# Corleno/Nonstationary_Multivariate_Gaussian_Process

Hardware: AMD Instinct MI355X
Metric: log-posterior evals/sec (N=2048, D=3 nonseparable GP) (higher is better)
Workload: dtype f64

## Files before the change

nonstationary_multivariate_gaussian_process_amd/csrc/nmgp_chol.hip:

```cpp
#include "nmgp_internal.h"
#include <cstring>

namespace nmgpk {

static inline int cdiv_c(long long a, long long b) { return (int)((a + b - 1) / b); }

typedef double v4d __attribute__((ext_vector_type(4)));

#define SY_BM 128
#define SY_BK 16
#define SY_LD (SY_BM + 16)
#define SY_SB 8

__device__ __forceinline__ int clamp_row_pair(int r, int rows) {
    int rc = r < rows - 1 ? r : rows - 2;
    return rc < 0 ? 0 : rc;
}

__device__ __forceinline__ double fast_recip(double p) {
    double x = __builtin_amdgcn_rcp(p);
    double e = fma(-p, x, 1.0);
    x = fma(x, e, x);
    e = fma(-p, x, 1.0);
    x = fma(x, e, x);
// ... 47 lines not shown
    potf2_step<KC, 2>(a, colbuf, pivs, nb, info, goff, r, g, tid);
    potf2_step<KC, 3>(a, colbuf, pivs, nb, info, goff, r, g, tid);
}

__device__ __forceinline__ void potf2_body(double* __restrict__ A, int lda, int nb, int* __restrict__ info, int goff, int tid,
                                           double (*colbuf)[64], double* pivs) {
    const int r = tid & 63, g = (tid >> 6) & 3;
    double a[16];
#pragma unroll
    for (int kk = 0; kk < 16; ++kk) {
        const int c = 4 * kk + g;
        double v = (r == c) ? 1.0 : 0.0;
        if (r < nb && c <= r) v = A[(size_t)c * lda + r];
        a[kk] = v;
    }
    if (tid < 64) pivs[tid] = 1.0;
    if (g == 0) colbuf[0][r] = a[0];
    __syncthreads();
#define PF(K) potf2_steps4<K>(a, colbuf, pivs, nb, info, goff, r, g, tid)
    PF(0); PF(1); PF(2); PF(3); PF(4); PF(5); PF(6); PF(7); PF(8); PF(9); PF(10); PF(11); PF(12); PF(13); PF(14); PF(15);
#undef PF
    __syncthreads();
#pragma unroll
    for (int kk = 0; kk < 16; ++kk) {
        const int c = 4 * kk + g;
        if (r < nb && c <= r) A[(size_t)c * lda + r] = a[kk] * rsqrt(pivs[c]);
    }
}

typedef double v2d __attribute__((ext_vector_type(2)));
typedef int v4i __attribute__((ext_vector_type(4)));

__device__ __forceinline__ void syrk_fused_first_block(double* lds, const v4d (&acc)[2][2][2], bool owner, int wj,
                                                       double* __restrict__ C, int ldc, int* __restrict__ info, int goff);

#define SY_SMEM (4 * SY_BK * SY_LD)
#define SCHUR_PATCH (32 * 33)
#define SY_SCHUR_SMEM (8 * SCHUR_PATCH + 6 * 256)
static_assert(SY_SCHUR_SMEM >= SY_SMEM && SY_SCHUR_SMEM * 8 * 2 <= 160 * 1024, "Schur epilogue LDS");

template <int M>
__device__ __forceinline__ double svc_schur_value(double sigma2, int a, int b, bool rc, const double* __restrict__ Lr, double il2,
                                                  const double* __restrict__ Lc, double kv, double nai, double gcb) {
    constexpr int UR = M <= 3 ? 8 : 1;
    const double gra = sigma2 * Lr[a * (a + 1) / 2] * il2;
    double s = 0.0;
#pragma unroll UR
    for (int q = 1; q <= b; ++q) s += Lr[a * (a + 1) / 2 + q] * Lc[b * (b + 1) / 2 + q];
    double v = kv * s;
    if (rc) v += sigma2 * ((a == b ? 1.0 : 0.0) + Lr[a * (a + 1) / 2] * Lr[b * (b + 1) / 2] * il2);
    v += gra * nai * gcb;
    return v;
}

template <int M, bool ALLB>
__device__ __forceinline__ void svc_schur_entries(const SchurEpi& e, double sigma2, int r, const double* __restrict__ Lr, double il2,
                                                  int c, double kv, double nai, const double* gc) {
    constexpr int T = M * (M + 1) / 2;
    constexpr int UR = M <= 3 ? 8 : 1;
    const size_t Ns = (size_t)e.N;
    const double* __restrict__ Lc = e.Lv + (size_t)c * T;
    const double lcc = M <= 4 ? 0.0 : Lc[0];
#pragma unroll UR
    for (int a = 1; a < M; ++a) {
#pragma unroll UR
        for (int b = 1; b <= (ALLB ? a : a - 1); ++b) {
            const double gcb = M <= 4 ? gc[b - 1] : sigma2 * Lc[b * (b + 1) / 2] / (lcc * lcc);
// ... 71 lines not shown
                        const double* Lc = e.Lv + (size_t)c * T_;
                        P[il * 33 + jl] = svc_schur_value<M>(sigma2, 2, 1, false, Lc, gc[M - 1], Lr, kv, nai, gt[(128 + r - row0) * GS]);
                    }
                } else {
                    svc_schur_entries<M, false>(e, sigma2, r, Lr, il2, c, kv, nai, gc);
                }
            }
        }
        __builtin_amdgcn_wave_barrier();
    }
}

template <int M>
__device__ __forceinline__ void svc_schur_yrow(const SchurEpi& e, int i) {
    constexpr int T = M * (M + 1) / 2;
    if (i >= e.N) return;
    const size_t Ns = (size_t)e.N;
    const int n1 = (M - 1) * e.N;
    const double sigma2 = exp(e.tse[0]);
    const double* Li = e.Lv + (size_t)i * T;
    const double l00 = Li[0];
    const double il2 = 1.0 / (l00 * l00);
    const double vi = e.y[i] / l00;
    const double r = vi - (sigma2 * il2) * e.u[i];
#pragma unroll
    for (int a = 1; a < M; ++a) e.S[((size_t)(a - 1) * Ns + i) * e.ld + n1] = e.y[(size_t)a * Ns + i] - Li[a * (a + 1) / 2] * r;
}

template <int SM = 0>
__device__ __forceinline__ void syrk_tile_fast(const double* __restrict__ A, int lda, double* __restrict__ C, int ldc, int K,
                                               int row0, int col0, bool diag, int kt0, bool beta0, int ncw, int yrow,
                                               int nyr, double* sA0, double* sB0, bool skip00 = false,
                                               int* __restrict__ finfo = nullptr, int fgoff = 0, bool mirror = false,
                                               int fresh0 = 0x7fffffff, const SchurEpi* se = nullptr) {
    constexpr int BK = 16;
    constexpr int SBUF = BK * SY_LD;
    const int tid = threadIdx.x, lane = tid & 63, w = tid >> 6;
    const int wi = w & 1, wj = w >> 1;
    const int l15 = lane & 15, l4 = lane >> 4;
    const int rp = tid & 63, cg = tid >> 6;
    const int offA = (cg * lda + row0 + 2 * rp) * 8, offB = (cg * lda + col0 + 2 * rp) * 8;
    const __amdgpu_buffer_rsrc_t rsrc = __builtin_amdgcn_make_buffer_rsrc((void*)A, 0, 0x7fffffff, 0x00020000);
    const int gstep = BK * lda * 8, ghalf = 8 * lda * 8;
    int soff = kt0 * gstep;
    const bool has_y = diag && yrow >= 0;
    const bool ywave = has_y && wi == 0 && wj >= 2;
    const int offY = ((tid & 15) * lda + yrow + (tid >> 4)) * 8;
    double* sY = sB0;
    v4i ra0, ra1, rb0, rb1;
    double ry = 0.0;
    auto gload = [&]() {
        ra0 = __builtin_amdgcn_raw_buffer_load_b128(rsrc, offA, soff, 0);
        ra1 = __builtin_amdgcn_raw_buffer_load_b128(rsrc, offA, soff + ghalf, 0);
        if (!diag) {
            rb0 = __builtin_amdgcn_raw_buffer_load_b128(rsrc, offB, soff, 0);
            rb1 = __builtin_amdgcn_raw_buffer_load_b128(rsrc, offB, soff + ghalf, 0);
        }
        if (has_y && tid < 16 * nyr) {
            typedef int v2i __attribute__((ext_vector_type(2)));
            const v2i t2 = __builtin_amdgcn_raw_buffer_load_b64(rsrc, offY, soff, 0);
            ry = __builtin_bit_cast(double, t2);
        }
        soff += gstep;
    };
    double* wA = sA0 + cg * SY_LD + 2 * rp;
    double* wB = sB0 + cg * SY_LD + 2 * rp;
    auto sstore = [&](int buf) {
// ... 138 lines not shown
#pragma unroll
            for (int r = 0; r < 4; ++r) {
                const int i = row0 + wi * 64 + 32 * p + 2 * l15;
                const int j = col0 + wj * 32 + 2 * (l4 + 4 * r) + tj;
                if (diag && j > i + 1) continue;
                double2 c;
                c.x = -acc[p][0][tj][r];
                c.y = -acc[p][1][tj][r];
                if (diag && j == i + 1) C[(size_t)j * ldc + i + 1] = c.y;
                else *reinterpret_cast<double2*>(&C[(size_t)j * ldc + i]) = c;
            }
    }
    if (mirror && active) {
        double* T = sA0 + w * (32 * 33);
        const int jl = lane & 31, ih = lane >> 5;
#pragma unroll
        for (int p = 0; p < 2; ++p) {
#pragma unroll
            for (int sx = 0; sx < 2; ++sx)
#pragma unroll
                for (int tj = 0; tj < 2; ++tj)
#pragma unroll
                    for (int r = 0; r < 4; ++r) T[(2 * l15 + sx) * 33 + 2 * (l4 + 4 * r) + tj] = -acc[p][sx][tj][r];
            const int rowm = col0 + wj * 32 + jl;
#pragma unroll
            for (int q = 0; q < 16; ++q) {
                const int il = 2 * q + ih;
                const int colm = row0 + wi * 64 + 32 * p + il;
                const double v = T[il * 33 + jl];
                if (colm > rowm) C[(size_t)colm * ldc + rowm] = v;
            }
        }
    }
    if (finfo != nullptr) syrk_fused_first_block(sA0, acc, fowner, wj, C, ldc, finfo, fgoff);
}

template <int NWJ, int BK, int SM = 0>
__device__ __forceinline__ void syrk_tile_body(const double* __restrict__ A, int lda, double* __restrict__ C, int ldc, int mrows,
                                               int ncols, int K, long long bstride, long long cstride, int ktri, int swz,
                                               int nbatch, int bx, int by, int bz0, double* sAb, double* sBb,
                                               int tri_row0 = 0x7fffffff, int tri_k0 = 0, int* __restrict__ finfo = nullptr,
                                               int fistride = 0, int fgoff = 0, const SchurEpi* sep = nullptr) {
    const int nyr = (ktri >> 2) & 31;
    const bool skipq = (ktri & 128) != 0;
    const bool mirror = (ktri & 512) != 0;
    const bool rowmajor = (ktri & 1024) != 0;
    const int yrow = nyr ? mrows : -1;
    (void)rowmajor;
    ktri &= 1;
    const int fresh0 = tri_row0 == 0x7fffffff ? 0x7fffffff : tri_row0 + tri_k0;
    constexpr int NT = 128 * NWJ;
    constexpr int CW = 128 / NWJ;
    constexpr int TJ = CW / 16;
    constexpr int NQ = (64 * BK) / NT;
    constexpr int CGS = NT / 64;
    double (*sA)[BK * SY_LD] = reinterpret_cast<double (*)[BK * SY_LD]>(sAb);
    double (*sB)[BK * SY_LD] = reinterpret_cast<double (*)[BK * SY_LD]>(sBb);
    int bi = bx, bj = by;
    int bz = bz0;
    if (swz) {
        const int t = bx, q = t >> 3;
        const int tiles_pm = swz > 0 ? swz : -swz;
        const long long g = swz > 0 ? ((long long)(q >> 6) * 8 + (t & 7)) * 64 + (q & 63) : (long long)t;
        int idx;
        if (finfo != nullptr) {
            if (g >= (long long)tiles_pm * nbatch) return;
            if (g < nbatch) {
                bz = (int)g;
                idx = 0;
            } else {
                const long long g2 = g - nbatch;
                bz = (int)(g2 / (tiles_pm - 1));
                idx = 1 + (int)(g2 - (long long)bz * (tiles_pm - 1));
            }
        } else {
            bz = (int)(g / tiles_pm);
            if (bz >= nbatch) return;
            idx = (int)(g - (long long)bz * tiles_pm);
        }
// ... 41 lines not shown
    bi = __builtin_amdgcn_readfirstlane(bi);
    bj = __builtin_amdgcn_readfirstlane(bj);
    bz = __builtin_amdgcn_readfirstlane(bz);
    A += (size_t)bz * bstride;
    C += (size_t)bz * cstride;
    SchurEpi se{};
    if constexpr (SM > 0) {
        static_assert(NWJ == 4 && BK == 16, "the Schur epilogue assumes 8 waves of 64 x 32");
        constexpr int T = SM * (SM + 1) / 2;
        se = *sep;
        se.x += (size_t)(bz / se.cps) * se.xstride;
        se.y += (size_t)(bz / se.cps) * se.ystride;
        se.ell += (size_t)bz * se.N;
        se.Lv += (size_t)bz * se.N * T;
        se.tse += (size_t)bz * ((size_t)se.N * (1 + T) + 1);
        se.u += (size_t)bz * se.N;
        se.S += (size_t)bz * se.bstride;
    }
    const bool diag = (bi == bj);
    const int tid = threadIdx.x, lane = tid & 63, w = tid >> 6;
    const int wi = w & 1, wj = w >> 1;
    const int row0 = bi * SY_BM, col0 = bj * SY_BM;
    if constexpr (NWJ == 4 && BK == 16) {
        const int ncw = ncols - col0 >= SY_BM ? SY_BM : ncols - col0;
        if (row0 + SY_BM <= mrows && (ncw == SY_BM || ncw == 64) && col0 + SY_BM <= mrows && (K & 31) == 0 &&
            (long long)(K + 16) * lda * 8 < 0x7fff0000LL) {
            int kt0f = ktri ? row0 / BK : 0;
            if (row0 >= tri_row0) {
                const int z = (row0 - tri_row0 - tri_k0) / BK;
                kt0f = z > 0 ? (z & ~1) : 0;
            }
            syrk_tile_fast<SM>(A, lda, C, ldc, K, row0, col0, diag, kt0f, ktri != 0, ncw, yrow, nyr, &sA[0][0], &sB[0][0],
                               skipq && bi == 0 && bj == 0, (finfo != nullptr && bi == 0 && bj == 0) ? finfo + (size_t)bz * fistride : nullptr,
                               fgoff, mirror, fresh0, &se);
            return;
        }
    }
    const int rp = tid & 63, cg = tid >> 6;
    double2 ra[NQ], rb[NQ];

    const int ri = row0 + 2 * rp, rj = col0 + 2 * rp;
    const int ric = clamp_row_pair(ri, mrows), rjc = clamp_row_pair(rj, mrows);
    const bool ix = ri < mrows, iy = ri + 1 < mrows, jx = rj < mrows, jy = rj + 1 < mrows;
    const bool ish = ix && (ric != ri), jsh = jx && (rjc != rj);
    auto gload = [&](int k0) {
#pragma unroll
        for (int q = 0; q < NQ; ++q) {
            const int kc = k0 + cg + CGS * q;
            const double* colp = A + (size_t)(kc < K ? kc : K - 1) * lda;
            ra[q] = *reinterpret_cast<const double2*>(colp + ric);
            if (!diag) rb[q] = *reinterpret_cast<const double2*>(colp + rjc);
        }
    };
    auto sstore = [&](int buf, int k0) {
#pragma unroll
        for (int q = 0; q < NQ; ++q) {
            const int kl = cg + CGS * q;
            const bool kin = (k0 + kl) < K;
            double2 va, vb;
            va.x = (kin && ix) ? (ish ? ra[q].y : ra[q].x) : 0.0;
            va.y = (kin && iy) ? ra[q].y : 0.0;
            *reinterpret_cast<double2*>(&sA[buf][kl * SY_LD + 2 * rp]) = va;
            if (!diag) {
                vb.x = (kin && jx) ? (jsh ? rb[q].y : rb[q].x) : 0.0;
                vb.y = (kin && jy) ? rb[q].y : 0.0;
                *reinterpret_cast<double2*>(&sB[buf][kl * SY_LD + 2 * rp]) = vb;
            }
// ... 355 lines not shown
            for (int r = 0; r < 4; ++r) {
                const int a = l4 + 4 * r, b = l15;
                Sr[r] = (a >= b) ? P.S[(16 * i + b) * PB_LD + 16 * i + a] : P.S[(16 * i + a) * PB_LD + 16 * i + b];
            }
#pragma unroll
            for (int kk = 0; kk < 4; ++kk) Sr = __builtin_amdgcn_mfma_f64_16x16x4f64(-Xown[kk], Xown[kk], Sr, 0, 0, 0);
        } else if (w < 3 && i < 4) {
            Xown = solve_rows(q, i);
            for (int j = q + 1; j <= i; ++j) {
                const v4d xj = (j == i) ? Xown : solve_rows(q, j);
                v4d acc;
#pragma unroll
                for (int reg = 0; reg < 4; ++reg) acc[reg] = P.S[(16 * j + l4 + 4 * reg) * PB_LD + 16 * i + l15];
#pragma unroll
                for (int kk = 0; kk < 4; ++kk) acc = __builtin_amdgcn_mfma_f64_16x16x4f64(-xj[kk], Xown[kk], acc, 0, 0, 0);
#pragma unroll
                for (int reg = 0; reg < 4; ++reg) P.S[(16 * j + l4 + 4 * reg) * PB_LD + 16 * i + l15] = acc[reg];
            }
        }
    }
    __syncthreads();
}

__device__ __forceinline__ void potf2b_store(double* __restrict__ A, int lda, int nb, const Potf2Lds& P, int tid, int nthreads) {
    for (int idx = tid; idx < 4096; idx += nthreads) {
        const int r = idx & 63, c = idx >> 6;
        if (r < nb && c < nb) {
            if (c <= r) A[(size_t)c * lda + r] = P.S[c * PB_LD + r];
            else if ((c >> 4) == (r >> 4)) A[(size_t)c * lda + r] = P.Einv[c >> 4][c & 15][r & 15];
        }
    }
}

__device__ __forceinline__ void syrk_fused_first_block(double* lds, const v4d (&acc)[2][2][2], bool owner, int wj,
                                                       double* __restrict__ C, int ldc, int* __restrict__ info, int goff) {
    static_assert(sizeof(Potf2Lds) <= 4 * SY_BK * SY_LD * sizeof(double), "the block's LDS must fit the operand buffers");
    Potf2Lds& P = *reinterpret_cast<Potf2Lds*>(lds);
    const int tid = threadIdx.x, lane = tid & 63;
    const int l15 = lane & 15, l4 = lane >> 4;
    for (int idx = tid; idx < 4096; idx += (int)blockDim.x) {
        const int r = idx & 63, c = idx >> 6;
        if (c > r) P.S[c * PB_LD + r] = 0.0;
    }
    if (owner) {
#pragma unroll
        for (int p = 0; p < 2; ++p)
#pragma unroll
            for (int sx = 0; sx < 2; ++sx)
#pragma unroll
                for (int tj = 0; tj < 2; ++tj)
#pragma unroll
                    for (int r = 0; r < 4; ++r) {
                        const int i = 32 * p + 2 * l15 + sx;
                        const int j = 32 * wj + 2 * (l4 + 4 * r) + tj;
                        if (i >= j) P.S[j * PB_LD + i] = -acc[p][sx][tj][r];
                    }
    }
    __syncthreads();
    potf2b_core_mfma(P, info, goff);
    potf2b_store(C, ldc, 64, P, tid, (int)blockDim.x);
}

__global__ __launch_bounds__(256) void k_potf2_64b(double* __restrict__ A, int lda, int nb, int* __restrict__ info,
                                                    int goff, long long bstride, int istride) {
    A += (size_t)blockIdx.x * bstride;
    info += (size_t)blockIdx.x * istride;
    __shared__ Potf2Lds P;
    const int tid = threadIdx.x;
#pragma unroll
    for (int k = 0; k < 16; ++k) {
        const int idx = tid + 256 * k;
        const int r = idx & 63, c = idx >> 6;
        double v = (r == c) ? 1.0 : 0.0;
        if (r < nb && c <= r) v = A[(size_t)c * lda + r];
        P.S[c * PB_LD + r] = v;
    }
    __syncthreads();
    potf2b_core_mfma(P, info, goff);
    potf2b_store(A, lda, nb, P, tid, 256);
}

static void potf2_64(hipStream_t s, double* A, int lda, int nb, int* info, int goff, int batch, long long bstride,
                     int istride, bool precise) {
    if (precise)
        NMGP_LAUNCH(k_potf2_64, dim3(batch), dim3(256), 0, s, A, lda, nb, info, goff, bstride, istride);
    else
        NMGP_LAUNCH(k_potf2_64b, dim3(batch), dim3(256), 0, s, A, lda, nb, info, goff, bstride, istride);
}

#define SS_LD 80
__global__ __launch_bounds__(256) void k_syrk_small(const double* __restrict__ A, int lda, double* __restrict__ C, int ldc,
                                                     int mrows, int ncols, int K, long long bstride, int tiles_pm, int nbatch,
                                                     int tri_row0, int tri_k0, int* __restrict__ info, int istride, int goff) {
// ... 109 lines not shown
            if (c > r) P.S[c * PB_LD + r] = 0.0;
        }
        if (active) {
#pragma unroll
            for (int tj = 0; tj < 2; ++tj)
#pragma unroll
                for (int ti = 0; ti < 2; ++ti)
#pragma unroll
                    for (int r = 0; r < 4; ++r) {
                        const int i = wi * 32 + ti * 16 + l15;
                        const int j = wj * 32 + tj * 16 + l4 + 4 * r;
                        if (i >= j) P.S[j * PB_LD + i] = acc[tj][ti][r];
                    }
        }
        __syncthreads();
        potf2b_core_mfma(P, info + (size_t)bz * istride, goff);
        potf2b_store(C, ldc, 64, P, tid, 256);
        return;
    }
    if (active) {
#pragma unroll
        for (int tj = 0; tj < 2; ++tj)
#pragma unroll
            for (int ti = 0; ti < 2; ++ti)
#pragma unroll
                for (int r = 0; r < 4; ++r) {
                    const int i = row0 + wi * 32 + ti * 16 + l15;
                    const int j = col0 + wj * 32 + tj * 16 + l4 + 4 * r;
                    if (i < mrows && j < ncols && i >= j) C[(size_t)j * ldc + i] = acc[tj][ti][r];
                }
    }
}

bool syrk_lower(hipStream_t s, const double* A, int lda, double* C, int ldc, int mrows, int ncols, int K, int batch,
                long long bstride, long long cstride, int ktri, int tri_row0, int tri_k0, int* finfo, int fistride, int goff,
                const SyrkHook* hook) {
    if (mrows <= 0 || ncols <= 0 || K <= 0) return false;
    const SyrkPlan pl = syrk_plan(lda, ldc, mrows, ncols, K, batch, ktri, false, tri_row0 != kNoTriRows);
    const long long cs = cstride < 0 ? bstride : cstride;
    void* tok = nullptr;
    if (hook && hook->begin) {
        const double elems = (double)ncols * mrows - 0.5 * (double)ncols * (ncols - 1);
        tok = hook->begin(hook->user, s, 2.0 * K * elems * batch, 8.0 * batch * (2.0 * elems + (double)mrows * K));
    }
    bool fused;
    if (!ktri && K >= 128 && batch <= 16 && (long long)pl.tiles * batch <= switches().syrk_small_max && cs == bstride &&
        (lda & 1) == 0 && mrows >= 2) {
        const int gx = (mrows + 63) / 64, gy = (ncols + 63) / 64;
        int tiles = 0;
        for (int bj = 0; bj < gy; ++bj) tiles += gx - bj > 0 ? gx - bj : 0;
        fused = finfo != nullptr && mrows >= 64 && ncols >= 64;
        NMGP_LAUNCH(k_syrk_small, dim3((unsigned)(tiles * batch)), dim3(256), 0, s, A, lda, C, ldc, mrows, ncols, K, bstride, tiles,
                    batch, tri_row0, tri_k0, fused ? finfo : (int*)nullptr, fistride, goff);
    } else {
        fused = finfo != nullptr && !ktri && cs == bstride && pl.mrows >= SY_BM && (ncols >= SY_BM || ncols == 64) &&
                (K & 31) == 0 && (long long)(K + 16) * lda * 8 < 0x7fff0000LL;
        SyrkPlan pf = pl;
        if (fused && pf.swz == 0) {
            pf.grid = dim3((unsigned)((long long)pf.tiles * batch), 1, 1);
            pf.swz = -pf.tiles;
        }
        NMGP_LAUNCH(k_syrk_lower, pf.grid, dim3(512), 0, s, A, lda, C, ldc, pf.mrows, ncols, K, bstride, cs, pf.kflags,
                    pf.swz, batch, tri_row0, tri_k0, fused ? finfo : (int*)nullptr, fistride, goff);
    }
    if (tok && hook->end) hook->end(hook->user, tok);
    return fused;
}

int syrk_schur(hipStream_t s, const double* X, int lda, int N, int M, int batch, const SchurEpi& e) {
    if (N <= 0) return 0;
    if (M < 2 || M > 8) return NMGP_E_UNSUPPORTED;
    const SyrkPlan pl = syrk_plan(lda, lda, N, N, N, batch, 2, false);
    switch (M) {
#define SCHUR_CASE(m) \
        case m: NMGP_LAUNCH(k_syrk_schur<m>, pl.grid, dim3(512), 0, s, X, lda, pl.mrows, e.bstride, pl.kflags, pl.swz, batch, e); break;
        SCHUR_CASE(2) SCHUR_CASE(3) SCHUR_CASE(4) SCHUR_CASE(5) SCHUR_CASE(6) SCHUR_CASE(7) SCHUR_CASE(8)
#undef SCHUR_CASE
    }
    return 0;
}


template <int SRC>
__device__ inline double quad_bcast(double v) {
    constexpr int ctrl = SRC | (SRC << 2) | (SRC << 4) | (SRC << 6);
    int lo = __double2loint(v), hi = __double2hiint(v);
    lo = __builtin_amdgcn_mov_dpp(lo, ctrl, 0xF, 0xF, true);
    hi = __builtin_amdgcn_mov_dpp(hi, ctrl, 0xF, 0xF, true);
    return __hiloint2double(hi, lo);
}

template <int KC, int GC>
__device__ __forceinline__ void trsm_step(double (&x)[16], const double (*Lm)[65], const double* rinv, int g) {
    constexpr int c = 4 * KC + GC;
    double xc = x[KC] * rinv[c];
    xc = quad_bcast<GC>(xc);
    if (g == GC) x[KC] = xc;
    double t[16];
#pragma unroll
// ... 482 lines not shown
    __syncthreads();
    PS_STAMP(5);
    if (isC) {
#pragma unroll
        for (int sg = 0; sg < 4; ++sg)
#pragma unroll
            for (int kk = 0; kk < 4; ++kk)
#pragma unroll
                for (int q = 0; q < 4; ++q) {
                    const double a = -Xs[(16 * q + l15) * PS_XLD + 16 * sg + 4 * kk + l4];
                    Un[q] = __builtin_amdgcn_mfma_f64_16x16x4f64(a, Tk[sg][kk], Un[q], 0, 0, 0);
                }
    }
    Potf2Lds& P = *reinterpret_cast<Potf2Lds*>(smem);
    __syncthreads();
    if (isC) {
#pragma unroll
        for (int q = 0; q < 4; ++q)
#pragma unroll
            for (int r = 0; r < 4; ++r) {
                const int rr = 16 * w + l15, cc = 16 * q + 4 * r + l4;
                P.S[cc * PB_LD + rr] = (cc <= rr) ? Un[q][r] : 0.0;
            }
    }
    __syncthreads();
    PS_STAMP(6);
    potf2b_core_mfma(P, info + (size_t)by * istride, ck + 64);
    PS_STAMP(7);
    potf2b_store(A + (size_t)(ck + 64) * lda + (ck + 64), lda, 64, P, tid, 512);
    PS_STAMP(8);
#undef PS_STAMP
}

__global__ void k_set_row(double* __restrict__ A, int lda, int row, const double* __restrict__ v, int n,
                          long long bstride, long long vstride, int cps) {
    int j = blockIdx.x * blockDim.x + threadIdx.x;
    if (j < n) A[(size_t)blockIdx.y * bstride + (size_t)j * lda + row] = v[(size_t)(blockIdx.y / cps) * vstride + j];
}
void set_row(hipStream_t s, double* A, int lda, int row, const double* v, int n, int batch, long long bstride,
             long long vstride, int cps) {
    NMGP_LAUNCH(k_set_row, dim3(cdiv_c(n, 256), batch), dim3(256), 0, s, A, lda, row, v, n, bstride, vstride, cps < 1 ? 1 : cps);
}
__global__ void k_get_row(const double* __restrict__ A, int lda, int row, double* __restrict__ v, int n,
                          long long bstride, long long vstride) {
    int j = blockIdx.x * blockDim.x + threadIdx.x;
    if (j < n) v[(size_t)blockIdx.y * vstride + j] = A[(size_t)blockIdx.y * bstride + (size_t)j * lda + row];
}
void get_row(hipStream_t s, const double* A, int lda, int row, double* v, int n, int batch, long long bstride,
             long long vstride) {
    NMGP_LAUNCH(k_get_row, dim3(cdiv_c(n, 256), batch), dim3(256), 0, s, A, lda, row, v, n, bstride, vstride);
}

struct Factorisation {
    hipStream_t s, s2;
    double* A;
    int lda, n, extra, xtri;
    int* info;
    int batch;
    long long bs;
    int is;
    bool precise;
    const SyrkHook* hook;
    long long* stamps;
    bool block_done = false;

    double* at(int row, int col) const { return A + (size_t)col * lda + row; }
    int active_rows(int cend) const { return n + extra + (cend < xtri ? cend : xtri); }
    bool take_block_done() {
        const bool done = block_done;
        block_done = false;
        return done;
    }

    void update(hipStream_t st, int c0, int k, int c1, int ncols, int fuse_width) {
        const bool fuse = fuse_width >= 64 && !precise;
        const bool done = syrk_lower(st, at(c1, c0), lda, at(c1, c1), lda, active_rows(c0 + k) - c1, ncols, k, batch, bs, -1, 0,
                                     xtri > 0 ? n + extra - c1 : kNoTriRows, c0, fuse ? info : nullptr, is, c1, hook);
        if (fuse) block_done = done;
    }

    void block_solve(int c0, int w) {
        if (!take_block_done()) potf2_64(s, at(c0, c0), lda, w, info, c0, batch, bs, is, precise);
        trsm_64(s, at(c0, c0), lda, w, at(c0 + w, c0), lda, active_rows(c0 + w) - (c0 + w), batch, bs, precise);
    }

    void fused_steps(int c0, int w, bool leaf) {
        if (!take_block_done()) potf2_64(s, at(c0, c0), lda, 64, info, c0, batch, bs, is, precise);
        const int nk = w / 64;
        for (int k = 0; k < nk; ++k) {
            const int ck = c0 + 64 * k;
            const int m_act = active_rows(ck + 64);
            const int rows = m_act - (ck + 64);
            if (rows <= 0) continue;
            const int has_prev = k > 0, has_next = k + 1 < nk;
            const int T = 1 + (rows > 64 ? cdiv_c(rows - 64, 128) : 0);
            SyrkPlan pl;
            const int u_m = m_act - (ck + 128), u_n = c0 + w - (ck + 128);
            if (has_prev && u_m > 0 && u_n > 0) pl = syrk_plan(lda, lda, u_m, u_n, 64, 1, 0, true);
            const int pre = (ck + 192 <= c0 + w) ? 1 : 0;
            if (pre) pl.kflags |= 128;
            long long* st = stamps ? stamps + (size_t)(ck / 64) * 16 : nullptr;
            const int un_fresh = xtri > 0 ? n + extra + (has_prev ? ck - 64 : ck) : kNoTriRows;
            const int u_tri = xtri > 0 ? n + extra - 64 * NMGP_XTRI_SEED_BLOCKS : kNoTriRows;
            if (leaf && pl.tiles == 0 && !pre && nk == 2) {
                if (k == 0)
                    NMGP_LAUNCH((k_panel_step<1, 4>), dim3((unsigned)(T * batch)), dim3(512), 0, s, A, lda, ck, 0, 1, m_act, c0 + w, bs, info,
                                is, T, 0, 0, 0, 0, batch, 0, un_fresh, u_tri, st);
                else
                    NMGP_LAUNCH((k_panel_step<2, 6>), dim3((unsigned)(T * batch)), dim3(512), 0, s, A, lda, ck, 1, 0, m_act, c0 + w, bs, info,
                                is, T, 0, 0, 0, 0, batch, 0, un_fresh, u_tri, st);
            } else {
                NMGP_LAUNCH((k_panel_step<0, 2>), dim3((unsigned)((T + pl.tiles) * batch)), dim3(512), 0, s, A, lda, ck, has_prev, has_next, m_act,
                            c0 + w, bs, info, is, T, pl.mrows, u_n, pl.kflags, pl.tiles, batch, pre, un_fresh, u_tri, st);
            }
        }
    }

    void panel_rl(int c0, int w) {
        for (int j0 = c0; j0 < c0 + w; j0 += 64) {
            const int jb = (c0 + w - j0 < 64) ? (c0 + w - j0) : 64;
            block_solve(j0, jb);
            update(s, j0, jb, j0 + jb, c0 + w - (j0 + jb), c0 + w - (j0 + jb));
        }
    }

    enum Leaf {
        kBlockSolve,
        kFusedSteps,
        kLeaf128
    };
    void panel_halving(int c0, int w, int base, Leaf leaf) {
        if (w <= base) {
            if (leaf == kBlockSolve || (leaf == kLeaf128 && w != 128)) block_solve(c0, w);
            else fused_steps(c0, w, leaf == kLeaf128);
            return;
        }
        int h = ((w / 2 + 63) / 64) * 64;
        if (h >= w) h = ((w - 1) / 64) * 64;
        panel_halving(c0, h, base, leaf);
        update(s, c0, h, c0 + h, w - h, w - h);
        panel_halving(c0 + h, w - h, base, leaf);
    }

    void panel(int c0, int w) {
        const Switches& sw = switches();
        const bool mfma_ok = w > 0 && (w % 64 == 0) && (lda % 2 == 0) && !precise;
        const bool small = sw.fused_max_batch >= 0 ? batch <= sw.fused_max_batch : (long long)batch * n <= 73728;
        const int rec_min_batch = 4;
        if (mfma_ok && (sw.panel == Switches::kFused || (sw.panel == Switches::kAuto && small)))
            panel_halving(c0, w, fused_base(w), kFusedSteps);
        else if (mfma_ok && sw.panel == Switches::kAuto && batch >= rec_min_batch && w >= 128)
            panel_halving(c0, w, 128, kLeaf128);
        else if (sw.panel == Switches::kRl || (sw.panel != Switches::kRec && batch < rec_min_batch))
            panel_rl(c0, w);
        else
            panel_halving(c0, w, 64, kBlockSolve);
    }
    int fused_base(int w) const {
        if (switches().fused_base >= 64) return switches().fused_base;
        if (w > 256 && (batch >= 16 || (xtri > 0 && batch >= 5))) return 256;
        return w;
    }

    void run(int nb1, hipEvent_t* ev) {
        const bool la = (s2 != nullptr && ev != nullptr && n > 2 * nb1 && batch <= switches().la_max_batch && !precise);
        if (!la) {
            for (int c0 = 0; c0 < n; c0 += nb1) {
                const int w1 = (n - c0 < nb1) ? (n - c0) : nb1;
                const int c1 = c0 + w1;
                panel(c0, w1);
                update(s, c0, w1, c1, n - c1, n - c1 < nb1 ? n - c1 : nb1);
            }
            return;
        }
        hipEventRecord(ev[0], s);
        hipStreamWaitEvent(s2, ev[0], 0);
        int k = 0;
        bool prevB = false;
        for (int c0 = 0; c0 < n; c0 += nb1, ++k) {
            const int w1 = (n - c0 < nb1) ? (n - c0) : nb1;
            const int c1 = c0 + w1;
            const int w1n = (c1 < n) ? ((n - c1 < nb1) ? (n - c1) : nb1) : 0;
            const int c2 = c1 + w1n;
            hipEvent_t evPanel = ev[1 + 2 * k], evB = ev[2 + 2 * k];
            panel(c0, w1);
            if (c1 >= n) break;
            if (prevB) hipStreamWaitEvent(s, ev[2 + 2 * (k - 1)], 0);
            update(s, c0, w1, c1, w1n, w1n);
            hipEventRecord(evPanel, s);
            prevB = false;
            if (c2 < n) {
                hipStreamWaitEvent(s2, evPanel, 0);
                update(s2, c0, w1, c2, n - c2, 0);
                hipEventRecord(evB, s2);
                prevB = true;
            }
        }
        if (prevB) hipStreamWaitEvent(s, ev[2 + 2 * (k - 1)], 0);
    }
};

void potrf_lower(hipStream_t s, hipStream_t s2, hipEvent_t* ev, double* A, int lda, int n, int extra, int xtri,
                 int nb1, int* info, int batch, long long bstride, int istride, const SyrkHook* hook, int precise) {
    if (nb1 <= 0)
        nb1 = (batch >= 16 && n >= 4096) ? 2048
              : (((batch >= 4 && n >= 4096) || (batch >= 32 && n >= 2048)) && (long long)batch * n > 73728) ? 1024 : 512;
    const int nsteps = (n + 63) / 64;
    Factorisation f{s, s2, A, lda, n, extra, xtri, info, batch, bstride, istride, precise != 0, hook, g_step_stamps.begin(s, nsteps)};
    f.run(nb1, ev);
    g_step_stamps.dump(s, nsteps);
}

static_assert(SY_BM + 2 * SY_BK - 2 <= 64 * NMGP_XTRI_SEED_BLOCKS, "update tiles of L^-T rows would read left of the seeded band");
static_assert(NMGP_XTRI_SEED_BLOCKS == 3, "k_panel_step (u_tri) and k_xtri_seed's grid (4 column blocks per row block) assume three seeded blocks");
__global__ __launch_bounds__(256) void k_xtri_seed(double* __restrict__ A, int lda, int row0, int n, int pad,
                                                    long long bstride) {
    A += (size_t)blockIdx.z * bstride;
    const int lane = threadIdx.x & 63, w = threadIdx.x >> 6;
    if (blockIdx.x == gridDim.x - 1) {
        for (int c = blockIdx.y * 256 + threadIdx.x; c < n; c += 256 * gridDim.y)
            for (int q = 0; q < pad; ++q) A[(size_t)c * lda + row0 + q] = 0.0;
// ... 18 lines not shown
```

nonstationary_multivariate_gaussian_process_amd/csrc/nmgp_internal.h:

```cpp
#pragma once

#include <hip/hip_runtime.h>
#include <rocblas/rocblas.h>
#include <rocsolver/rocsolver.h>

#include <cmath>
#include <cstdio>
#include <cstdlib>
#include <cstring>
#include <map>
#include <string>
#include <utility>
#include <vector>

#include "nmgp.h"

#define NMGP_JITTER 1e-6
#define NMGP_PRECISION 1e-6

struct DevBuf {
    double* p = nullptr;
    size_t cap = 0;
};

// ... 315 lines not shown
void pred_rows_reduce(hipStream_t st, const double* A, int ld, int n, int R0, int zrow, int E, double* part, double* mean,
                      double* colsq);
void svc_predvar(hipStream_t st, const double* Lstar, const double* colsq, int S, int M, const double* tse,
                 double* var);
void sep_crossvec(hipStream_t st, int mode, const double* x, const double* sig, const double* ell, int N,
                  const double* xs, const double* tl_star, const double* ts_star, double sig0, double l0, int S,
                  double* KX);
void sep_predict(hipStream_t st, const double* Cq, const double* a, const double* wB, const double* VB, int M,
                 const double* wK, int N, double sigma2, const double* Bdiag, const double* kss, bool strict_clip, int S,
                 double* mean, double* var);
void sep_predict_chol(hipStream_t st, const double* dots, const double* sqs, const double* wB, const double* VB, int M, double sigma2,
                      const double* Bdiag, const double* kss, bool strict_clip, int S, double* mean, double* var);
void cols_to_rows(hipStream_t st, const double* KX, int N, int S, double* A, int ld, int R0, int batch, long long bstride);
void sep_star(hipStream_t st, const double* proj, int S, double mu_l, double mu_s, double* tl_star, double* ts_star,
              double* kss);
void add_diag(hipStream_t s, double* A, int ld, int n, double v);
void rotate_y(hipStream_t s, const double* Y, const double* VB, int N, int M, double* yt);
void sep_blocks(hipStream_t s, const double* K, const double* wB, const double* sigma2p, int N, int M, double* out,
                int ldo, long long bstride);
#define NMGP_SEP_TR_G 128
int sep_traces(hipStream_t s, const double* Cneg, const double* K, const double* alpha, int N, int M, double* out);
void weighted_sum_lower(hipStream_t s, const double* Cneg, const double* wB, int N, int M, double* C);
void sep_prep_b(hipStream_t s, const double* pars, long long P, const double* Y, const double* small, int small_per, int N, int M,
                double* ell, double* sig, double* yt, int B);
void sep_blocks_b(hipStream_t s, const double* x, const double* ell, const double* sig, const double* small, int small_per, int N, int M,
                  double* S, int ldo, long long bstride, double* Kout, int B);
void sep_reduce_b(hipStream_t s, const double* Cneg, const double* K, const double* alpha, const double* small, int small_per, int N,
                  int M, int G, double* C, double* out, double* xi, int B);
void sep_adjoint_b(hipStream_t s, const double* x, const double* ell, const double* sig, const double* U, const double* small,
                   int small_per, int M, const double* C, int N, double* part, double* g, int B);
void two_col_rhs_b(hipStream_t s, const double* pars, long long P, double mu_a, double mu_b, int N, double* R, int B);
void ps_rows_reduce(hipStream_t s, const double* A, int ld, long long bstride, int n, int R0, int zrow, int E, double* part,
                    int batch, double* dots, double* sqs, long long ostride, long long o0);
bool syrk_lower(hipStream_t s, const double* A, int lda, double* C, int ldc, int mrows, int ncols, int K, int batch,
                long long bstride, long long cstride = -1, int ktri = 0, int tri_row0 = 0x7fffffff, int tri_k0 = 0,
                int* finfo = nullptr, int fistride = 0, int goff = 0, const SyrkHook* hook = nullptr);
struct SchurEpi {
    const double* x;
    const double* ell;
    const double* Lv;
    const double* tse;
    const double* y;
    const double* u;
    double* S;
    int ld;
    int N;
    int xstride;
    int cps;
    long long ystride;
    long long bstride;
};
int syrk_schur(hipStream_t s, const double* X, int lda, int N, int M, int batch, const SchurEpi& e);
void identity_rows(hipStream_t s, double* A, int lda, int row0, int n, int pad, int batch = 1, long long bstride = 0);
void set_row(hipStream_t s, double* A, int lda, int row, const double* v, int n, int batch, long long bstride,
             long long vstride, int cps = 1);
void get_row(hipStream_t s, const double* A, int lda, int row, double* v, int n, int batch, long long bstride,
             long long vstride);
void potrf_lower(hipStream_t s, hipStream_t s2, hipEvent_t* ev, double* A, int lda, int n, int extra, int xtri,
                 int nb1, int* info, int batch, long long bstride, int istride, const SyrkHook* hook = nullptr,
                 int precise = 0);

}
```

Measured before the change: 1694.

## Add fused 128-column leaf kernels for throughput Cholesky panels

Adds k_leaf_diag128 and k_leaf128, which factor a 128-wide diagonal block and solve the panel rows below it with f64 MFMA triangular solves in a single launch. The SYRK epilogue can now factor the whole 128-column diagonal block instead of only 64, and a width-256 leaf is split into two 128 leaves with an update between them. This is meant to cut kernel launches and global round trips in the batched throughput schedule. It adds a lot of control flow and larger LDS use, and it only applies when the kLeaf128 schedule is selected.

Result: faster. 1714, median of 6 (+1.2%).

```diff
diff --git a/nonstationary_multivariate_gaussian_process_amd/csrc/nmgp_chol.hip b/nonstationary_multivariate_gaussian_process_amd/csrc/nmgp_chol.hip
--- a/nonstationary_multivariate_gaussian_process_amd/csrc/nmgp_chol.hip
+++ b/nonstationary_multivariate_gaussian_process_amd/csrc/nmgp_chol.hip
@@ -103,7 +103,8 @@
 typedef int v4i __attribute__((ext_vector_type(4)));
 
 __device__ __forceinline__ void syrk_fused_first_block(double* lds, const v4d (&acc)[2][2][2], bool owner, int wj,
-                                                       double* __restrict__ C, int ldc, int* __restrict__ info, int goff);
+                                                       double* __restrict__ C, int ldc, int* __restrict__ info, int goff,
+                                                       bool whole128);
 
 #define SY_SMEM (4 * SY_BK * SY_LD)
 #define SCHUR_PATCH (32 * 33)
@@ -241,7 +242,7 @@
                                                int row0, int col0, bool diag, int kt0, bool beta0, int ncw, int yrow,
                                                int nyr, double* sA0, double* sB0, bool skip00 = false,
                                                int* __restrict__ finfo = nullptr, int fgoff = 0, bool mirror = false,
-                                               int fresh0 = 0x7fffffff, const SchurEpi* se = nullptr) {
+                                               int fresh0 = 0x7fffffff, const SchurEpi* se = nullptr, bool f128 = false) {
     constexpr int BK = 16;
     constexpr int SBUF = BK * SY_LD;
     const int tid = threadIdx.x, lane = tid & 63, w = tid >> 6;
@@ -446,7 +447,7 @@
             }
         }
     }
-    if (finfo != nullptr) syrk_fused_first_block(sA0, acc, fowner, wj, C, ldc, finfo, fgoff);
+    if (finfo != nullptr) syrk_fused_first_block(sA0, acc, fowner, wj, C, ldc, finfo, fgoff, f128);
 }
 
 template <int NWJ, int BK, int SM = 0>
@@ -459,6 +460,7 @@
     const bool skipq = (ktri & 128) != 0;
     const bool mirror = (ktri & 512) != 0;
     const bool rowmajor = (ktri & 1024) != 0;
+    const bool f128 = (ktri & 2048) != 0;
     const int yrow = nyr ? mrows : -1;
     (void)rowmajor;
     ktri &= 1;
@@ -566,7 +568,7 @@
             }
             syrk_tile_fast<SM>(A, lda, C, ldc, K, row0, col0, diag, kt0f, ktri != 0, ncw, yrow, nyr, &sA[0][0], &sB[0][0],
                                skipq && bi == 0 && bj == 0, (finfo != nullptr && bi == 0 && bj == 0) ? finfo + (size_t)bz * fistride : nullptr,
-                               fgoff, mirror, fresh0, &se);
+                               fgoff, mirror, fresh0, &se, f128);
             return;
         }
     }
@@ -988,8 +990,116 @@
     }
 }
 
+__device__ __forceinline__ void trsm_ops_load(const double* __restrict__ L, int lda, int tid, double (&ot)[5]) {
+#pragma unroll
+    for (int j = 0; j < 5; ++j) {
+        const int idx = tid + 512 * j;
+        const int blk = idx >> 8, kk = (idx >> 6) & 3, l = idx & 63;
+        const int rr = l & 15, kc = 4 * kk + (l >> 4);
+        double v;
+        if (blk < 6) {
+            const int q = blk == 0 ? 1 : (blk < 3 ? 2 : 3);
+            const int pp = blk == 0 ? 0 : (blk < 3 ? blk - 1 : blk - 3);
+            v = -L[(size_t)(16 * pp + kc) * lda + 16 * q + rr];
+        } else {
+            const int q = blk - 6;
+            if (kc < rr) v = L[(size_t)(16 * q + rr) * lda + 16 * q + kc];
+            else if (kc == rr) v = 1.0 / L[(size_t)(16 * q + rr) * lda + 16 * q + rr];
+            else v = 0.0;
+        }
+        ot[j] = v;
+    }
+}
+__device__ __forceinline__ void trsm_ops_store(double* ops, int tid, const double (&ot)[5]) {
+#pragma unroll
+    for (int j = 0; j < 5; ++j) {
+        const int idx = tid + 512 * j;
+        const int blk = idx >> 8, kk = (idx >> 6) & 3, l = idx & 63;
+        ops[(blk * 64 + l) * 4 + kk] = ot[j];
+    }
+}
+__device__ __forceinline__ void trsm_solve64(v4d (&T)[4], const v4d* ops, int lane) {
+#pragma unroll
+    for (int pp = 0; pp < 4; ++pp) {
+        const v4d ai = ops[(6 + pp) * 64 + lane];
+        v4d x0 = {0.0, 0.0, 0.0, 0.0};
+#pragma unroll
+        for (int kk = 0; kk < 4; ++kk) x0 = __builtin_amdgcn_mfma_f64_16x16x4f64(ai[kk], T[pp][kk], x0, 0, 0, 0);
+        T[pp] = x0;
+#pragma unroll
+        for (int kk = 0; kk < 4; ++kk)
+#pragma unroll
+            for (int q = pp + 1; q < 4; ++q) {
+                const double a = reinterpret_cast<const double*>(&ops[((q == 1 ? 0 : (q == 2 ? 1 : 3)) + pp) * 64 + lane])[kk];
+                T[q] = __builtin_amdgcn_mfma_f64_16x16x4f64(a, T[pp][kk], T[q], 0, 0, 0);
+            }
+    }
+}
+
+#define LD_XLD 66
+#define LD_SMEM_DOUBLES (2560 + 64 * LD_XLD)
+static_assert(sizeof(Potf2Lds) <= LD_SMEM_DOUBLES * sizeof(double), "the factorisation's LDS aliases the solve's");
+__device__ __forceinline__ void leaf_diag_lower(double* __restrict__ D, int lda, int* __restrict__ info, int goff, double* smem) {
+    const int tid = threadIdx.x, lane = tid & 63, w = tid >> 6;
+    const int l15 = lane & 15, l4 = lane >> 4;
+    v4d* opsT = reinterpret_cast<v4d*>(smem);
+    double* Xs = smem + 2560;
+    const bool own = w < 4;
+    const int row = 64 + 16 * (w & 3) + l15;
+    double ot[5];
+    trsm_ops_load(D, lda, tid, ot);
+    v4d Tk[4], Un[4];
+#pragma unroll
+    for (int q = 0; q < 4; ++q)
+#pragma unroll
+        for (int r = 0; r < 4; ++r) {
+            const int c = 16 * q + 4 * r + l4;
+            Tk[q][r] = own ? D[(size_t)c * lda + row] : 0.0;
+            Un[q][r] = own ? D[(size_t)(64 + c) * lda + row] : 0.0;
+        }
+    trsm_ops_store(smem, tid, ot);
+    __syncthreads();
+    if (own) {
+        trsm_solve64(Tk, opsT, lane);
+#pragma unroll
+        for (int q = 0; q < 4; ++q)
+#pragma unroll
+            for (int r = 0; r < 4; ++r) {
+                D[(size_t)(16 * q + 4 * r + l4) * lda + row] = Tk[q][r];
+                Xs[(16 * w + l15) * LD_XLD + 16 * q + 4 * r + l4] = Tk[q][r];
+            }
+    }
+    __syncthreads();
+    if (own) {
+#pragma unroll
+        for (int sg = 0; sg < 4; ++sg)
+#pragma unroll
+            for (int kk = 0; kk < 4; ++kk)
+#pragma unroll
+                for (int q = 0; q < 4; ++q) {
+                    const double a = -Xs[(16 * q + l15) * LD_XLD + 16 * sg + 4 * kk + l4];
+                    Un[q] = __builtin_amdgcn_mfma_f64_16x16x4f64(a, Tk[sg][kk], Un[q], 0, 0, 0);
+                }
+    }
+    Potf2Lds& P = *reinterpret_cast<Potf2Lds*>(smem);
+    __syncthreads();
+    if (own) {
+#pragma unroll
+        for (int q = 0; q < 4; ++q)
+#pragma unroll
+            for (int r = 0; r < 4; ++r) {
+                const int rr = 16 * w + l15, cc = 16 * q + 4 * r + l4;
+                P.S[cc * PB_LD + rr] = (cc <= rr) ? Un[q][r] : 0.0;
+            }
+    }
+    __syncthreads();
+    potf2b_core_mfma(P, info, goff + 64);
+    potf2b_store(D + (size_t)64 * lda + 64, lda, 64, P, tid, 512);
+}
+
 __device__ __forceinline__ void syrk_fused_first_block(double* lds, const v4d (&acc)[2][2][2], bool owner, int wj,
-                                                       double* __restrict__ C, int ldc, int* __restrict__ info, int goff) {
+                                                       double* __restrict__ C, int ldc, int* __restrict__ info, int goff,
+                                                       bool whole128) {
     static_assert(sizeof(Potf2Lds) <= 4 * SY_BK * SY_LD * sizeof(double), "the block's LDS must fit the operand buffers");
     Potf2Lds& P = *reinterpret_cast<Potf2Lds*>(lds);
     const int tid = threadIdx.x, lane = tid & 63;
@@ -1015,6 +1125,11 @@
     __syncthreads();
     potf2b_core_mfma(P, info, goff);
     potf2b_store(C, ldc, 64, P, tid, (int)blockDim.x);
+    if (whole128) {
+        static_assert(LD_SMEM_DOUBLES <= 4 * SY_BK * SY_LD, "the 128-column diagonal block's LDS must fit the operand buffers");
+        __syncthreads();
+        leaf_diag_lower(C, ldc, info, goff, lds);
+    }
 }
 
 __global__ __launch_bounds__(256) void k_potf2_64b(double* __restrict__ A, int lda, int nb, int* __restrict__ info,
@@ -1190,10 +1305,10 @@
     }
 }
 
-bool syrk_lower(hipStream_t s, const double* A, int lda, double* C, int ldc, int mrows, int ncols, int K, int batch,
-                long long bstride, long long cstride, int ktri, int tri_row0, int tri_k0, int* finfo, int fistride, int goff,
-                const SyrkHook* hook) {
-    if (mrows <= 0 || ncols <= 0 || K <= 0) return false;
+int syrk_lower(hipStream_t s, const double* A, int lda, double* C, int ldc, int mrows, int ncols, int K, int batch,
+               long long bstride, long long cstride, int ktri, int tri_row0, int tri_k0, int* finfo, int fistride, int goff,
+               const SyrkHook* hook, int fuse_cols) {
+    if (mrows <= 0 || ncols <= 0 || K <= 0) return 0;
     const SyrkPlan pl = syrk_plan(lda, ldc, mrows, ncols, K, batch, ktri, false, tri_row0 != kNoTriRows);
     const long long cs = cstride < 0 ? bstride : cstride;
     void* tok = nullptr;
@@ -1202,6 +1317,7 @@
         tok = hook->begin(hook->user, s, 2.0 * K * elems * batch, 8.0 * batch * (2.0 * elems + (double)mrows * K));
     }
     bool fused;
+    bool whole = false;
     if (!ktri && K >= 128 && batch <= 16 && (long long)pl.tiles * batch <= switches().syrk_small_max && cs == bstride &&
         (lda & 1) == 0 && mrows >= 2) {
         const int gx = (mrows + 63) / 64, gy = (ncols + 63) / 64;
@@ -1214,6 +1330,8 @@
         fused = finfo != nullptr && !ktri && cs == bstride && pl.mrows >= SY_BM && (ncols >= SY_BM || ncols == 64) &&
                 (K & 31) == 0 && (long long)(K + 16) * lda * 8 < 0x7fff0000LL;
         SyrkPlan pf = pl;
+        whole = fused && fuse_cols == 128 && ncols >= SY_BM;
+        if (whole) pf.kflags |= 2048;
         if (fused && pf.swz == 0) {
             pf.grid = dim3((unsigned)((long long)pf.tiles * batch), 1, 1);
             pf.swz = -pf.tiles;
@@ -1222,7 +1340,7 @@
                     pf.swz, batch, tri_row0, tri_k0, fused ? finfo : (int*)nullptr, fistride, goff);
     }
     if (tok && hook->end) hook->end(hook->user, tok);
-    return fused;
+    return fused ? (whole ? 128 : 64) : 0;
 }
 
 int syrk_schur(hipStream_t s, const double* X, int lda, int N, int M, int batch, const SchurEpi& e) {
@@ -1771,6 +1889,100 @@
 #undef PS_STAMP
 }
 
+__global__ __launch_bounds__(512) void k_leaf_diag128(double* __restrict__ Ab, int lda, int ck, int have64, long long bstride,
+                                                       int* __restrict__ info, int istride) {
+    __shared__ __attribute__((aligned(32))) double smem[LD_SMEM_DOUBLES];
+    double* D = Ab + (size_t)blockIdx.x * bstride + (size_t)ck * lda + ck;
+    info += (size_t)blockIdx.x * istride;
+    const int tid = threadIdx.x;
+    if (!have64) {
+        Potf2Lds& P = *reinterpret_cast<Potf2Lds*>(smem);
+#pragma unroll
+        for (int k = 0; k < 8; ++k) {
+            const int idx = tid + 512 * k;
+            const int r = idx & 63, c = idx >> 6;
+            P.S[c * PB_LD + r] = (c <= r) ? D[(size_t)c * lda + r] : 0.0;
+        }
+        __syncthreads();
+        potf2b_core_mfma(P, info, ck);
+        potf2b_store(D, lda, 64, P, tid, 512);
+        __syncthreads();
+    }
+    leaf_diag_lower(D, lda, info, ck, smem);
+}
+
+#define LF_OPST0 4096
+#define LF_OPST1 (LF_OPST0 + 2560)
+#define LF_SMEM_DOUBLES (LF_OPST1 + 2560)
+__global__ __launch_bounds__(512, 4) void k_leaf128(double* __restrict__ Ab, int lda, int ck, int m_act0, int m_act,
+                                                     long long bstride, int nbatch, int un_fresh) {
+    __shared__ __attribute__((aligned(32))) double smem[LF_SMEM_DOUBLES];
+    const int tid = threadIdx.x, lane = tid & 63, w = tid >> 6;
+    const int l15 = lane & 15, l4 = lane >> 4;
+    const int bx = (int)blockIdx.x / nbatch, by = (int)blockIdx.x - bx * nbatch;
+    double* A = Ab + (size_t)by * bstride;
+    const v4d* opsC = reinterpret_cast<const v4d*>(smem);
+    const v4d* opsT = reinterpret_cast<const v4d*>(smem + LF_OPST0);
+    const int row = ck + 128 + 128 * bx + 16 * w + l15;
+    const bool rv = row < m_act;
+    const int rowc = rv ? row : (m_act - 1);
+    const bool in0 = row < m_act0;
+    const bool fresh1 = row >= un_fresh && row - un_fresh < 64;
+    double oc[8], ot[2][5];
+    v4d T0[4], T1[4];
+    const double* Lp = A + (size_t)ck * lda;
+#pragma unroll
+    for (int j = 0; j < 8; ++j) {
+        const int e = tid + 512 * j, q = e >> 10, sx = (e >> 6) & 15, l = e & 63;
+        oc[j] = -Lp[(size_t)(4 * sx + (l >> 4)) * lda + ck + 64 + 16 * q + (l & 15)];
+    }
+    trsm_ops_load(A + (size_t)ck * lda + ck, lda, tid, ot[0]);
+    trsm_ops_load(A + (size_t)(ck + 64) * lda + ck + 64, lda, tid, ot[1]);
+#pragma unroll
+    for (int q = 0; q < 4; ++q)
+#pragma unroll
+        for (int r = 0; r < 4; ++r) {
+            const int c = 16 * q + 4 * r + l4;
+            T0[q][r] = rv ? A[(size_t)(ck + c) * lda + rowc] : 0.0;
+            T1[q][r] = (rv && !fresh1) ? A[(size_t)(ck + 64 + c) * lda + rowc] : 0.0;
+        }
+#pragma unroll
+    for (int j = 0; j < 8; ++j) {
+        const int e = tid + 512 * j, q = e >> 10, sx = (e >> 6) & 15, l = e & 63;
+        smem[((q * 4 + (sx >> 2)) * 64 + l) * 4 + (sx & 3)] = oc[j];
+    }
+    trsm_ops_store(smem + LF_OPST0, tid, ot[0]);
+    trsm_ops_store(smem + LF_OPST1, tid, ot[1]);
+    __syncthreads();
+    trsm_solve64(T0, opsT, lane);
+    if (rv && in0) {
+#pragma unroll
+        for (int q = 0; q < 4; ++q)
+#pragma unroll
+            for (int r = 0; r < 4; ++r) A[(size_t)(ck + 16 * q + 4 * r + l4) * lda + row] = T0[q][r];
+    }
+    if (!in0) {
+#pragma unroll
+        for (int q = 0; q < 4; ++q) T0[q] = v4d{0.0, 0.0, 0.0, 0.0};
+    }
+#pragma unroll
+    for (int sg = 0; sg < 4; ++sg)
+#pragma unroll
+        for (int kk = 0; kk < 4; ++kk)
+#pragma unroll
+            for (int q = 0; q < 4; ++q) {
+                const double a = reinterpret_cast<const double*>(&opsC[(q * 4 + sg) * 64 + lane])[kk];
+                T1[q] = __builtin_amdgcn_mfma_f64_16x16x4f64(a, T0[sg][kk], T1[q], 0, 0, 0);
+            }
+    trsm_solve64(T1, opsT + 10 * 64, lane);
+    if (rv) {
+#pragma unroll
+        for (int q = 0; q < 4; ++q)
+#pragma unroll
+            for (int r = 0; r < 4; ++r) A[(size_t)(ck + 64 + 16 * q + 4 * r + l4) * lda + row] = T1[q][r];
+    }
+}
+
 __global__ void k_set_row(double* __restrict__ A, int lda, int row, const double* __restrict__ v, int n,
                           long long bstride, long long vstride, int cps) {
     int j = blockIdx.x * blockDim.x + threadIdx.x;
@@ -1801,30 +2013,41 @@
     bool precise;
     const SyrkHook* hook;
     long long* stamps;
-    bool block_done = false;
+    int block_done = 0;
 
     double* at(int row, int col) const { return A + (size_t)col * lda + row; }
     int active_rows(int cend) const { return n + extra + (cend < xtri ? cend : xtri); }
-    bool take_block_done() {
-        const bool done = block_done;
-        block_done = false;
+    int take_block_done() {
+        const int done = block_done;
+        block_done = 0;
         return done;
     }
 
-    void update(hipStream_t st, int c0, int k, int c1, int ncols, int fuse_width) {
+    void update(hipStream_t st, int c0, int k, int c1, int ncols, int fuse_width, bool leaf256 = false) {
         const bool fuse = fuse_width >= 64 && !precise;
-        const bool done = syrk_lower(st, at(c1, c0), lda, at(c1, c1), lda, active_rows(c0 + k) - c1, ncols, k, batch, bs, -1, 0,
-                                     xtri > 0 ? n + extra - c1 : kNoTriRows, c0, fuse ? info : nullptr, is, c1, hook);
+        const int done = syrk_lower(st, at(c1, c0), lda, at(c1, c1), lda, active_rows(c0 + k) - c1, ncols, k, batch, bs, -1, 0,
+                                    xtri > 0 ? n + extra - c1 : kNoTriRows, c0, fuse ? info : nullptr, is, c1, hook,
+                                    leaf256 ? 128 : 64);
         if (fuse) block_done = done;
     }
 
+    void leaf128(int ck) {
+        const int done = take_block_done();
+        if (done < 128) NMGP_LAUNCH(k_leaf_diag128, dim3((unsigned)batch), dim3(512), 0, s, A, lda, ck, done >= 64 ? 1 : 0, bs, info, is);
+        const int m_act = active_rows(ck + 128);
+        const int rows = m_act - (ck + 128);
+        if (rows <= 0) return;
+        NMGP_LAUNCH(k_leaf128, dim3((unsigned)(cdiv_c(rows, 128) * batch)), dim3(512), 0, s, A, lda, ck, active_rows(ck + 64), m_act, bs,
+                    batch, xtri > 0 ? n + extra + ck : kNoTriRows);
+    }
+
     void block_solve(int c0, int w) {
-        if (!take_block_done()) potf2_64(s, at(c0, c0), lda, w, info, c0, batch, bs, is, precise);
+        if (take_block_done() < 64) potf2_64(s, at(c0, c0), lda, w, info, c0, batch, bs, is, precise);
         trsm_64(s, at(c0, c0), lda, w, at(c0 + w, c0), lda, active_rows(c0 + w) - (c0 + w), batch, bs, precise);
     }
 
     void fused_steps(int c0, int w, bool leaf) {
-        if (!take_block_done()) potf2_64(s, at(c0, c0), lda, 64, info, c0, batch, bs, is, precise);
+        if (take_block_done() < 64) potf2_64(s, at(c0, c0), lda, 64, info, c0, batch, bs, is, precise);
         const int nk = w / 64;
         for (int k = 0; k < nk; ++k) {
             const int ck = c0 + 64 * k;
@@ -1868,33 +2091,53 @@
         kFusedSteps,
         kLeaf128
     };
+    static int left_width(int w) {
+        int h = ((w / 2 + 63) / 64) * 64;
+        if (h >= w) h = ((w - 1) / 64) * 64;
+        return h;
+    }
+    static bool starts_with_256(int w) {
+        while (w > 256) w = left_width(w);
+        return w == 256;
+    }
     void panel_halving(int c0, int w, int base, Leaf leaf) {
+        if (leaf == kLeaf128 && w == 256) {
+            leaf128(c0);
+            update(s, c0, 128, c0 + 128, 128, 128, true);
+            leaf128(c0 + 128);
+            return;
+        }
         if (w <= base) {
             if (leaf == kBlockSolve || (leaf == kLeaf128 && w != 128)) block_solve(c0, w);
             else fused_steps(c0, w, leaf == kLeaf128);
             return;
         }
-        int h = ((w / 2 + 63) / 64) * 64;
-        if (h >= w) h = ((w - 1) / 64) * 64;
+        const int h = left_width(w);
         panel_halving(c0, h, base, leaf);
-        update(s, c0, h, c0 + h, w - h, w - h);
+        update(s, c0, h, c0 + h, w - h, w - h, leaf == kLeaf128 && starts_with_256(w - h));
         panel_halving(c0 + h, w - h, base, leaf);
     }
 
-    void panel(int c0, int w) {
+    enum Sched { kSchedFused, kSchedThroughput, kSchedRl, kSchedRec };
+    Sched sched(int w) const {
         const Switches& sw = switches();
         const bool mfma_ok = w > 0 && (w % 64 == 0) && (lda % 2 == 0) && !precise;
         const bool small = sw.fused_max_batch >= 0 ? batch <= sw.fused_max_batch : (long long)batch * n <= 73728;
         const int rec_min_batch = 4;
-        if (mfma_ok && (sw.panel == Switches::kFused || (sw.panel == Switches::kAuto && small)))
-            panel_halving(c0, w, fused_base(w), kFusedSteps);
-        else if (mfma_ok && sw.panel == Switches::kAuto && batch >= rec_min_batch && w >= 128)
-            panel_halving(c0, w, 128, kLeaf128);
-        else if (sw.panel == Switches::kRl || (sw.panel != Switches::kRec && batch < rec_min_batch))
-            panel_rl(c0, w);
-        else
-            panel_halving(c0, w, 64, kBlockSolve);
-    }
+        if (mfma_ok && (sw.panel == Switches::kFused || (sw.panel == Switches::kAuto && small))) return kSchedFused;
+        if (mfma_ok && sw.panel == Switches::kAuto && batch >= rec_min_batch && w >= 128) return kSchedThroughput;
+        if (sw.panel == Switches::kRl || (sw.panel != Switches::kRec && batch < rec_min_batch)) return kSchedRl;
+        return kSchedRec;
+    }
+    void panel(int c0, int w) {
+        switch (sched(w)) {
+        case kSchedFused: panel_halving(c0, w, fused_base(w), kFusedSteps); break;
+        case kSchedThroughput: panel_halving(c0, w, 128, kLeaf128); break;
+        case kSchedRl: panel_rl(c0, w); break;
+        case kSchedRec: panel_halving(c0, w, 64, kBlockSolve); break;
+        }
+    }
+    bool panel_starts_with_256(int w) const { return w > 0 && sched(w) == kSchedThroughput && starts_with_256(w); }
     int fused_base(int w) const {
         if (switches().fused_base >= 64) return switches().fused_base;
         if (w > 256 && (batch >= 16 || (xtri > 0 && batch >= 5))) return 256;
@@ -1908,7 +2151,8 @@
                 const int w1 = (n - c0 < nb1) ? (n - c0) : nb1;
                 const int c1 = c0 + w1;
                 panel(c0, w1);
-                update(s, c0, w1, c1, n - c1, n - c1 < nb1 ? n - c1 : nb1);
+                const int wn = n - c1 < nb1 ? n - c1 : nb1;
+                update(s, c0, w1, c1, n - c1, wn, panel_starts_with_256(wn));
             }
             return;
         }
@@ -1925,7 +2169,7 @@
             panel(c0, w1);
             if (c1 >= n) break;
             if (prevB) hipStreamWaitEvent(s, ev[2 + 2 * (k - 1)], 0);
-            update(s, c0, w1, c1, w1n, w1n);
+            update(s, c0, w1, c1, w1n, w1n, panel_starts_with_256(w1n));
             hipEventRecord(evPanel, s);
             prevB = false;
             if (c2 < n) {
diff --git a/nonstationary_multivariate_gaussian_process_amd/csrc/nmgp_internal.h b/nonstationary_multivariate_gaussian_process_amd/csrc/nmgp_internal.h
--- a/nonstationary_multivariate_gaussian_process_amd/csrc/nmgp_internal.h
+++ b/nonstationary_multivariate_gaussian_process_amd/csrc/nmgp_internal.h
@@ -371,9 +371,9 @@
 void two_col_rhs_b(hipStream_t s, const double* pars, long long P, double mu_a, double mu_b, int N, double* R, int B);
 void ps_rows_reduce(hipStream_t s, const double* A, int ld, long long bstride, int n, int R0, int zrow, int E, double* part,
                     int batch, double* dots, double* sqs, long long ostride, long long o0);
-bool syrk_lower(hipStream_t s, const double* A, int lda, double* C, int ldc, int mrows, int ncols, int K, int batch,
-                long long bstride, long long cstride = -1, int ktri = 0, int tri_row0 = 0x7fffffff, int tri_k0 = 0,
-                int* finfo = nullptr, int fistride = 0, int goff = 0, const SyrkHook* hook = nullptr);
+int syrk_lower(hipStream_t s, const double* A, int lda, double* C, int ldc, int mrows, int ncols, int K, int batch,
+               long long bstride, long long cstride = -1, int ktri = 0, int tri_row0 = 0x7fffffff, int tri_k0 = 0,
+               int* finfo = nullptr, int fistride = 0, int goff = 0, const SyrkHook* hook = nullptr, int fuse_cols = 64);
 struct SchurEpi {
     const double* x;
     const double* ell;
```
